# e-sha/dvs_of_training_framework

Hardware: AMD Instinct MI355X
Metric: training samples/sec (256x256x5 event voxels) (higher is better)
Workload: dtype f32; 1 GPU; EV_FlowNet 256x256x5-bin synthetic events, batch 8 per GPU, fp32 (BASELINE.json configs[1]); full step: voxelise + fwd + multi-scale loss + bwd + AdamW-amsgrad; global_batch=8, parallelism=dp1

## Files before the change

dvs_of_training_framework_amd/csrc/fwd_min.hip:

```cpp
#include "conv_common.h"
#include <stdlib.h>

namespace {

constexpr unsigned FM_OOB = 0x80000000u;
constexpr int FM_NT = 512;
constexpr int FM_APA = 5;
constexpr int FM_AP = 8 * FM_APA;
constexpr int FM_AARR = FM_APA * 1024 + 16;

template <int NR>
struct FMGeom {
    static constexpr int PT = NR / 2;
    static constexpr int KS = 8 / PT;
    static constexpr int SLOTS = (NR + 2) * 18;
    static constexpr int BROWS = (SLOTS + 7) / 8;
    static constexpr int BPA = (BROWS + 7) / 8;
    static constexpr int BARR = BPA * 1024 + 16;
    static constexpr int BOFF = 8 * FM_AARR;
    static constexpr int NPIECE = FM_AP + 8 * BPA;
    static constexpr int LPW = NPIECE / 8;
    static constexpr int STAGE = ((8 * FM_AARR + 8 * BARR + 1023) / 1024) * 1024;
    static constexpr int XCH = 8 * 4 * 4096;
    static constexpr int LDS = 2 * STAGE > XCH ? 2 * STAGE : XCH;
};

__global__ __launch_bounds__(256) void min9_fwd_weights_kernel(const float *__restrict__ w, float *__restrict__ wt,
                                                               int Cout, int Ctot)
{
    const size_t i = (size_t)blockIdx.x * 256 + threadIdx.x;
    if (i >= (size_t)Cout * Ctot) return;
    const int ci = (int)(i % Ctot), co = (int)(i / Ctot);
    float k[3][3], r[3][3];
#pragma unroll
    for (int t = 0; t < 9; ++t) k[t / 3][t % 3] = w[((size_t)co * 9 + t) * Ctot + ci];
#pragma unroll
    for (int l = 0; l < 3; ++l) {
        r[0][l] = k[0][l];
        r[1][l] = (k[0][l] + k[1][l]) + k[2][l];
        r[2][l] = k[2][l];
    }
#pragma unroll
    for (int p = 0; p < 3; ++p) {
        const float v[3] = {r[p][0], (r[p][0] + r[p][1]) + r[p][2], r[p][2]};
#pragma unroll
        for (int q = 0; q < 3; ++q) wt[((size_t)(3 * p + q) * Cout + co) * Ctot + ci] = v[q];
    }
}

template <int NR, bool ZOUT>
__global__ __launch_bounds__(FM_NT) void fwd_min_f32_kernel(const GConvParams P)
{
#if defined(__HIP_DEVICE_COMPILE__)
    typedef FMGeom<NR> G;
    typedef float f32x2 __attribute__((ext_vector_type(2)));
    extern __shared__ __attribute__((aligned(1024))) unsigned char smem[];
    const int tid = threadIdx.x, lane = tid & 63;
    const int wave = __builtin_amdgcn_readfirstlane(tid >> 6);
    const int pt = wave % G::PT, ks = wave / G::PT;
    const int lrow = lane & 31, lh = lane >> 5;
    const int H = P.Hv, W = P.Wv;
    const int nbx = W / 16, nby = H / NR;

    unsigned wg = blockIdx.x;
    {
        const unsigned total = gridDim.x, x = wg & 7u, q = total >> 3, r = total & 7u;
        wg = x * q + min(x, r) + (wg >> 3);
    }
    const int nco = P.N / 32;
    const int cot = (int)(wg % (unsigned)nco), blk = (int)(wg / (unsigned)nco);
    const int co0 = 32 * cot;
    const int bx = blk % nbx, by = (blk / nbx) % nby, b = blk / (nbx * nby);
    const int oy = NR * by, ox = 16 * bx;

    const GSrc &S0 = P.src[0], &S1 = P.src[1];
    unsigned off_a[G::LPW], off_b[G::LPW - FM_APA];
#pragma unroll
    for (int i = 0; i < G::LPW; ++i) {
        const int p = wave + 8 * i;
        off_a[i] = FM_OOB;
        if (i >= FM_APA) off_b[i - FM_APA] = FM_OOB;
        if (i < FM_APA) {
            const int m = p / FM_APA, pp = p - FM_APA * m;
            const int j = 8 * pp + (lane >> 3);
            if (j < 36) {
                const int R = 8 * j + m;
                const int c = R >> 5, r = R & 31;
                off_a[i] = (unsigned)((((size_t)c * P.N + co0 + r) * P.Cin_tot + 4 * (lane & 7)) * 4);
            }
        } else {
            const int pb = p - FM_AP;
            const int m = pb / G::BPA, pp = pb - G::BPA * m;
            const int n = 8 * (8 * pp + (lane >> 3)) + m;
            if (n < G::SLOTS) {
                const int r = n / 18, c = n - 18 * r;
                if (((unsigned)(oy + r - 1) < (unsigned)H) & ((unsigned)(ox + c - 1) < (unsigned)W)) {
                    off_a[i] = (unsigned)((r * S0.sy + c * S0.sx + 4 * (lane & 7)) * 4);
                    off_b[i - FM_APA] = (unsigned)((r * S1.sy + c * S1.sx + 4 * (lane & 7)) * 4);
                }
            }
        }
    }
    const __amdgpu_buffer_rsrc_t wres = __builtin_amdgcn_make_buffer_rsrc((void *)P.W, 0, 0x7fffffff, 0x00020000);
    const __amdgpu_buffer_rsrc_t res0 = __builtin_amdgcn_make_buffer_rsrc(
        (void *)(S0.p - ((long long)S0.sy + S0.sx)), 0, 0x7fffffff, 0x00020000);
    const __amdgpu_buffer_rsrc_t res1 = __builtin_amdgcn_make_buffer_rsrc(
        (void *)(S1.p - ((long long)S1.sy + S1.sx)), 0, 0x7fffffff, 0x00020000);
    const int base0 = __builtin_amdgcn_readfirstlane(
        (int)(((long long)b * S0.sb + (long long)oy * S0.sy + (long long)ox * S0.sx) * 4));
    const int base1 = __builtin_amdgcn_readfirstlane(
        (int)(((long long)b * S1.sb + (long long)oy * S1.sy + (long long)ox * S1.sx) * 4));
    const int nch0 = S0.C / 32, nchunks = P.Cin_tot / 32;

    auto issue = [&](int stage_idx, int ch) {
        unsigned char *st = smem + stage_idx * G::STAGE;
        const bool m1 = ch >= nch0;
        const int so_w = ch * 128;
        const int so_x = m1 ? base1 + (ch - nch0) * 128 : base0 + ch * 128;
#pragma unroll
        for (int i = 0; i < G::LPW; ++i) {
            const int p = wave + 8 * i;
            if (i < FM_APA) {
                const int m = p / FM_APA, pp = p - FM_APA * m;
                __attribute__((address_space(3))) void *dst =
                    (__attribute__((address_space(3))) void *)(st + m * FM_AARR + pp * 1024);
                __builtin_amdgcn_raw_ptr_buffer_load_lds(wres, dst, 16, off_a[i], so_w, 0, 0);
            } else {
                const int pb = p - FM_AP;
                const int m = pb / G::BPA, pp = pb - G::BPA * m;
                __attribute__((address_space(3))) void *dst =
                    (__attribute__((address_space(3))) void *)(st + G::BOFF + m * G::BARR + pp * 1024);
                if (m1)
                    __builtin_amdgcn_raw_ptr_buffer_load_lds(res1, dst, 16, off_b[i - FM_APA], so_x, 0, 0);
                else
                    __builtin_amdgcn_raw_ptr_buffer_load_lds(res0, dst, 16, off_a[i], so_x, 0, 0);
            }
        }
    };

#ifndef FM_B64
    constexpr int FRAG = 16;
#else
    constexpr int FRAG = 8;
#endif
    const int abase = (lrow & 7) * FM_AARR + (lrow >> 3) * 128 + FRAG * lh;
    int bbase[9];
#pragma unroll
    for (int r = 0; r < 3; ++r)
#pragma unroll
        for (int c = 0; c < 3; ++c) {
            const int n = (2 * pt + (lrow >> 4) + r) * 18 + (lrow & 15) + c;
            bbase[3 * r + c] = G::BOFF + (n & 7) * G::BARR + (n >> 3) * 128 + FRAG * lh;
        }

    f32x16 acc[9];
#pragma unroll
    for (int c = 0; c < 9; ++c)
#pragma unroll
        for (int r = 0; r < 16; ++r) acc[c][r] = 0.f;

#ifndef FM_PROBE
#define FM_PROBE 0
#endif
    auto compute = [&](int u) {
        const unsigned char *st = smem + u * G::STAGE;
#ifdef FM_STAGGER
        if (wave >= 4) __builtin_amdgcn_s_sleep(FM_STAGGER);
#endif
#ifndef FM_B64
#pragma unroll
        for (int gi = 0; gi < 4 / G::KS; ++gi) {
            const int kg = ks + G::KS * gi;
            f32x4 x[9];
#pragma unroll
            for (int c = 0; c < 9; ++c) x[c] = *(const f32x4 *)(st + bbase[c] + 32 * kg);
            f32x4 an = *(const f32x4 *)(st + abase + 32 * kg);
            f32x4 rw[3][3], xt[9];
#pragma unroll
            for (int c = 0; c < 3; ++c) {
                rw[0][c] = x[c] - x[3 + c];
                rw[1][c] = x[3 + c];
                rw[2][c] = x[6 + c] - x[3 + c];
            }
#pragma unroll
            for (int p = 0; p < 3; ++p) {
                xt[3 * p] = rw[p][0] - rw[p][1];
                xt[3 * p + 1] = rw[p][1];
                xt[3 * p + 2] = rw[p][2] - rw[p][1];
            }
#pragma unroll
            for (int c = 0; c < 9; ++c) {
                const f32x4 ac = an;
                if (c + 1 < 9) an = *(const f32x4 *)(st + abase + (c + 1) * 512 + 32 * kg);
#pragma unroll
                for (int j = 0; j < 4; ++j)
                    acc[c] = __builtin_amdgcn_mfma_f32_32x32x2f32(ac[j], xt[c][j], acc[c], 0, 0, 0);
            }
        }
#else
#pragma unroll
        for (int gi = 0; gi < 8 / G::KS; ++gi) {
            const int kg = ks + G::KS * gi;
            f32x2 a[9], x[9];
#pragma unroll
            for (int c = 0; c < 9; ++c) a[c] = *(const f32x2 *)(st + abase + ((FM_PROBE & 2) ? 0 : c) * 512 + 16 * kg);
#pragma unroll
            for (int c = 0; c < 9; ++c) x[c] = *(const f32x2 *)(st + bbase[(FM_PROBE & 2) ? 0 : c] + 16 * kg);
            f32x2 rw[3][3], xt[9];
#pragma unroll
            for (int c = 0; c < 3; ++c) {
                rw[0][c] = x[c] - x[3 + c];
                rw[1][c] = x[3 + c];
                rw[2][c] = x[6 + c] - x[3 + c];
            }
#pragma unroll
            for (int p = 0; p < 3; ++p) {
                xt[3 * p] = rw[p][0] - rw[p][1];
                xt[3 * p + 1] = rw[p][1];
                xt[3 * p + 2] = rw[p][2] - rw[p][1];
            }
#pragma unroll
            for (int c = 0; c < 9; ++c) {
                acc[c] = __builtin_amdgcn_mfma_f32_32x32x2f32(a[c][0], xt[c][0], acc[c], 0, 0, 0);
                acc[c] = __builtin_amdgcn_mfma_f32_32x32x2f32(a[c][1], xt[c][1], acc[c], 0, 0, 0);
            }
        }
#endif
    };

    issue(0, 0);
    for (int ch = 0; ch < nchunks; ++ch) {
        asm volatile("s_waitcnt vmcnt(0)" ::: "memory");
        if (!(FM_PROBE & 4) || ch == 0) __builtin_amdgcn_s_barrier();
        if (ch + 1 < nchunks && (!(FM_PROBE & 1) || ch == 0)) issue((ch + 1) & 1, ch + 1);
        compute(ch & 1);
    }

    const int ecq = lane & 7;
    f32x4 bias4 = {0.f, 0.f, 0.f, 0.f};
    if (P.bias) bias4 = *(const f32x4 *)(P.bias + co0 + 4 * ecq);
    __builtin_amdgcn_s_barrier();
#pragma unroll
    for (int f = 0; f < 4; ++f) {
        const int fa = f >> 1, fb = f & 1;
        const f32x16 t = (acc[3 * fa + fb] + acc[3 * fa + fb + 1]) + (acc[3 * fa + 3 + fb] + acc[3 * fa + 4 + fb]);
        unsigned char *xt_ = smem + (wave * 4 + f) * 4096;
#pragma unroll
        for (int g = 0; g < 4; ++g) {
            const f32x4 v = {t[4 * g], t[4 * g + 1], t[4 * g + 2], t[4 * g + 3]};
            *(f32x4 *)(xt_ + lrow * 128 + (((2 * g + lh) ^ (lrow & 7)) << 4)) = v;
        }
    }
    __builtin_amdgcn_s_barrier();
    const GDst &D = P.dst[0];
#pragma unroll
    for (int fi = 0; fi < 4 / G::KS; ++fi) {
        const int f = ks + G::KS * fi;
        const int fa = f >> 1, fb = f & 1;
#pragma unroll
        for (int it = 0; it < 4; ++it) {
            const int px = 8 * it + (lane >> 3);
            const int xo = px * 128 + ((ecq ^ (px & 7)) << 4);
            f32x4 v = *(const f32x4 *)(smem + (pt * 4 + f) * 4096 + xo);
#pragma unroll
            for (int k = 1; k < G::KS; ++k) v += *(const f32x4 *)(smem + ((pt + G::PT * k) * 4 + f) * 4096 + xo);
            const int yy = oy + 2 * pt + (px >> 4), xx = ox + (px & 15);
            const long long o = (long long)b * D.sb + (long long)yy * D.sy + (long long)xx * D.sx +
                                (long long)fa * D.ph_y + (long long)fb * D.ph_x + co0 + 4 * ecq;
            v += bias4;
            if (P.bias_cls) {
                const int Y = 2 * yy + fa, X = 2 * xx + fb;
                const int cls = 3 * (Y == 0 ? 1 : Y == P.out_H - 1 ? 2 : 0) + (X == 0 ? 1 : X == P.out_W - 1 ? 2 : 0);
                if (cls) v += *(const f32x4 *)(P.bias_cls + cls * P.N + co0 + 4 * ecq);
            }
            if (ZOUT) *(f32x4 *)(P.zout + o) = v;
#pragma unroll
            for (int e = 0; e < 4; ++e) v[e] = act_fwd(v[e], P.act);
            *(f32x4 *)(D.p + o) = v;
        }
    }
#endif
}

}

bool min9_shape_ok(int mfma, int nsrc, const int *C, const int *nhwc, int Cout, int H, int W)
{
    static const bool off = getenv("DVSOF_NO_FWD_MIN") != nullptr;
    if (off || mfma != 0 || nsrc != 2) return false;
    for (int s = 0; s < 2; ++s)
        if (!nhwc[s] || (C[s] & 31)) return false;
    return (Cout & 31) == 0 && (W % 16) == 0 && (H % 4) == 0 && H >= 4;
}

int min9_prepare_fwd(const float *w, float *wt, int Cout, int Ctot, hipStream_t st)
{
    const size_t n = (size_t)Cout * Ctot;
    hipLaunchKernelGGL(min9_fwd_weights_kernel, dim3((unsigned)((n + 255) / 256)), dim3(256), 0, st, w, wt, Cout, Ctot);
    DVSOF_LAUNCH_CHECK();
    return DVSOF_OK;
}

template <int NR, bool ZOUT>
static int fm_launch(const GConvParams &P, int grid, hipStream_t st)
{
    typedef FMGeom<NR> G;
    static bool attr_set = false;
    if (!attr_set) {
        DVSOF_HIP_TRY(hipFuncSetAttribute((const void *)fwd_min_f32_kernel<NR, ZOUT>,
                                          hipFuncAttributeMaxDynamicSharedMemorySize, G::LDS));
        attr_set = true;
    }
    hipLaunchKernelGGL((fwd_min_f32_kernel<NR, ZOUT>), dim3(grid), dim3(FM_NT), G::LDS, st, P);
    DVSOF_LAUNCH_CHECK();
    conv_note_kernel(NR == 8 ? DVSOF_KERNEL_FWD_MIN8 : DVSOF_KERNEL_FWD_MIN4, 0);
    return DVSOF_OK;
}

int fwd_min_launch(const GConvParams &P, hipStream_t st)
{
    for (int s = 0; s < 2; ++s) {
        const GSrc &S = P.src[s];
        if (!S.p || (reinterpret_cast<uintptr_t>(S.p) & 15) || ((S.sb | S.sy | S.sx) & 3) || S.sc != 1) return DVSOF_EINVAL;
    }
    const GDst &D = P.dst[0];
    if (D.addend || D.addend2 || D.actsrc || D.sc != 1 || ((D.sb | D.sy | D.sx | D.ph_y | D.ph_x) & 3)) return DVSOF_EINVAL;
    if ((reinterpret_cast<uintptr_t>(D.p) & 15) || (reinterpret_cast<uintptr_t>(P.zout) & 15) ||
        (reinterpret_cast<uintptr_t>(P.W) & 15) || (reinterpret_cast<uintptr_t>(P.bias) & 15) ||
        (reinterpret_cast<uintptr_t>(P.bias_cls) & 15))
        return DVSOF_EINVAL;
    static const int force = getenv("DVSOF_FWD_MIN_NR") ? atoi(getenv("DVSOF_FWD_MIN_NR")) : 0;
    const long long per_row = (long long)P.B * (P.Wv / 16) * (P.N / 32);
    int nr = 4;
    if (P.Hv % 8 == 0 && per_row * (P.Hv / 8) >= 256) nr = 8;
    if ((force == 4 || force == 8) && P.Hv % force == 0) nr = force;
    const int grid = (int)(per_row * (P.Hv / nr));
    const bool z = P.zout != nullptr;
    if (nr == 8) return z ? fm_launch<8, true>(P, grid, st) : fm_launch<8, false>(P, grid, st);
    return z ? fm_launch<4, true>(P, grid, st) : fm_launch<4, false>(P, grid, st);
}
```

Baseline: 3263 samples/s.

## Stage 16-channel chunks through a four-deep LDS ring with software-pipelined MFMA

Shrinks each staged channel chunk from 32 to 16 channels and replaces the two-stage double buffer with a four-slot LDS ring, issuing loads two chunks ahead and waiting with a counted vmcnt instead of draining all loads. The compute is split into a load/Winograd-transform step and an MFMA step, and some waves lag the MFMA by one chunk so transforms and matrix work from different chunks interleave across waves. The weight and patch layouts in LDS are rebuilt for 4-row interleaving. This aims to hide global-to-LDS latency and barrier stalls, at the cost of more iterations, more barriers per channel, and more complex indexing that could introduce layout or bank-conflict issues.

```diff
diff --git a/dvs_of_training_framework_amd/csrc/fwd_min.hip b/dvs_of_training_framework_amd/csrc/fwd_min.hip
--- a/dvs_of_training_framework_amd/csrc/fwd_min.hip
+++ b/dvs_of_training_framework_amd/csrc/fwd_min.hip
@@ -5,24 +5,24 @@
 
 constexpr unsigned FM_OOB = 0x80000000u;
 constexpr int FM_NT = 512;
-constexpr int FM_APA = 5;
-constexpr int FM_AP = 8 * FM_APA;
-constexpr int FM_AARR = FM_APA * 1024 + 16;
+constexpr int FM_RING = 4;
+constexpr int FM_LPW = 4;
+constexpr int FM_STAGE = 8 * FM_LPW * 1024;
+constexpr int FM_AROWS = 72;
+constexpr int FM_AARR = FM_AROWS * 64 + 16;
+constexpr int FM_BOFF = ((4 * FM_AARR + 1023) / 1024) * 1024;
+constexpr int FM_WP = FM_BOFF / 1024;
 
 template <int NR>
 struct FMGeom {
     static constexpr int PT = NR / 2;
     static constexpr int KS = 8 / PT;
     static constexpr int SLOTS = (NR + 2) * 18;
-    static constexpr int BROWS = (SLOTS + 7) / 8;
-    static constexpr int BPA = (BROWS + 7) / 8;
-    static constexpr int BARR = BPA * 1024 + 16;
-    static constexpr int BOFF = 8 * FM_AARR;
-    static constexpr int NPIECE = FM_AP + 8 * BPA;
-    static constexpr int LPW = NPIECE / 8;
-    static constexpr int STAGE = ((8 * FM_AARR + 8 * BARR + 1023) / 1024) * 1024;
+    static constexpr int BROWS = ((SLOTS + 3) / 4 + 3) / 4 * 4;
+    static constexpr int BARR = BROWS * 64 + 16;
+    static_assert(FM_BOFF + 4 * BARR <= FM_STAGE, "the patch image overflows the stage");
     static constexpr int XCH = 8 * 4 * 4096;
-    static constexpr int LDS = 2 * STAGE > XCH ? 2 * STAGE : XCH;
+    static constexpr int LDS = FM_RING * FM_STAGE > XCH ? FM_RING * FM_STAGE : XCH;
 };
 
 __global__ __launch_bounds__(256) void min9_fwd_weights_kernel(const float *__restrict__ w, float *__restrict__ wt,
@@ -53,7 +53,6 @@
 {
 #if defined(__HIP_DEVICE_COMPILE__)
     typedef FMGeom<NR> G;
-    typedef float f32x2 __attribute__((ext_vector_type(2)));
     extern __shared__ __attribute__((aligned(1024))) unsigned char smem[];
     const int tid = threadIdx.x, lane = tid & 63;
     const int wave = __builtin_amdgcn_readfirstlane(tid >> 6);
@@ -74,29 +73,29 @@
     const int oy = NR * by, ox = 16 * bx;
 
     const GSrc &S0 = P.src[0], &S1 = P.src[1];
-    unsigned off_a[G::LPW], off_b[G::LPW - FM_APA];
-#pragma unroll
-    for (int i = 0; i < G::LPW; ++i) {
+    unsigned off_a[FM_LPW], off_b[FM_LPW];
+#pragma unroll
+    for (int i = 0; i < FM_LPW; ++i) {
         const int p = wave + 8 * i;
+        const int a = 1024 * p + 16 * lane;
         off_a[i] = FM_OOB;
-        if (i >= FM_APA) off_b[i - FM_APA] = FM_OOB;
-        if (i < FM_APA) {
-            const int m = p / FM_APA, pp = p - FM_APA * m;
-            const int j = 8 * pp + (lane >> 3);
-            if (j < 36) {
-                const int R = 8 * j + m;
+        off_b[i] = FM_OOB;
+        if (p < FM_WP) {
+            const int m = a / FM_AARR, o = a - FM_AARR * m;
+            if (m < 4 && o < FM_AROWS * 64) {
+                const int R = 4 * (o >> 6) + m;
                 const int c = R >> 5, r = R & 31;
-                off_a[i] = (unsigned)((((size_t)c * P.N + co0 + r) * P.Cin_tot + 4 * (lane & 7)) * 4);
+                off_a[i] = (unsigned)((((size_t)c * P.N + co0 + r) * P.Cin_tot + 4 * ((o >> 4) & 3)) * 4);
             }
         } else {
-            const int pb = p - FM_AP;
-            const int m = pb / G::BPA, pp = pb - G::BPA * m;
-            const int n = 8 * (8 * pp + (lane >> 3)) + m;
-            if (n < G::SLOTS) {
-                const int r = n / 18, c = n - 18 * r;
+            const int ab = a - FM_BOFF;
+            const int m = ab / G::BARR, o = ab - G::BARR * m;
+            const int n = 4 * (o >> 6) + m;
+            if (m < 4 && o < G::BROWS * 64 && n < G::SLOTS) {
+                const int r = n / 18, c = n - 18 * r, qq = (o >> 4) & 3;
                 if (((unsigned)(oy + r - 1) < (unsigned)H) & ((unsigned)(ox + c - 1) < (unsigned)W)) {
-                    off_a[i] = (unsigned)((r * S0.sy + c * S0.sx + 4 * (lane & 7)) * 4);
-                    off_b[i - FM_APA] = (unsigned)((r * S1.sy + c * S1.sx + 4 * (lane & 7)) * 4);
+                    off_a[i] = (unsigned)((r * S0.sy + c * S0.sx + 4 * qq) * 4);
+                    off_b[i] = (unsigned)((r * S1.sy + c * S1.sx + 4 * qq) * 4);
                 }
             }
         }
@@ -110,47 +109,35 @@
         (int)(((long long)b * S0.sb + (long long)oy * S0.sy + (long long)ox * S0.sx) * 4));
     const int base1 = __builtin_amdgcn_readfirstlane(
         (int)(((long long)b * S1.sb + (long long)oy * S1.sy + (long long)ox * S1.sx) * 4));
-    const int nch0 = S0.C / 32, nchunks = P.Cin_tot / 32;
-
-    auto issue = [&](int stage_idx, int ch) {
-        unsigned char *st = smem + stage_idx * G::STAGE;
+    const int nch0 = S0.C / 16, nchunks = P.Cin_tot / 16;
+
+    auto issue = [&](int u, int ch) {
+        unsigned char *st = smem + u * FM_STAGE;
         const bool m1 = ch >= nch0;
-        const int so_w = ch * 128;
-        const int so_x = m1 ? base1 + (ch - nch0) * 128 : base0 + ch * 128;
-#pragma unroll
-        for (int i = 0; i < G::LPW; ++i) {
+        const int so_w = __builtin_amdgcn_readfirstlane(ch * 64);
+        const int so_x = __builtin_amdgcn_readfirstlane(m1 ? base1 + (ch - nch0) * 64 : base0 + ch * 64);
+#pragma unroll
+        for (int i = 0; i < FM_LPW; ++i) {
             const int p = wave + 8 * i;
-            if (i < FM_APA) {
-                const int m = p / FM_APA, pp = p - FM_APA * m;
-                __attribute__((address_space(3))) void *dst =
-                    (__attribute__((address_space(3))) void *)(st + m * FM_AARR + pp * 1024);
+            __attribute__((address_space(3))) void *dst = (__attribute__((address_space(3))) void *)(st + 1024 * p);
+            if (p < FM_WP)
                 __builtin_amdgcn_raw_ptr_buffer_load_lds(wres, dst, 16, off_a[i], so_w, 0, 0);
-            } else {
-                const int pb = p - FM_AP;
-                const int m = pb / G::BPA, pp = pb - G::BPA * m;
-                __attribute__((address_space(3))) void *dst =
-                    (__attribute__((address_space(3))) void *)(st + G::BOFF + m * G::BARR + pp * 1024);
-                if (m1)
-                    __builtin_amdgcn_raw_ptr_buffer_load_lds(res1, dst, 16, off_b[i - FM_APA], so_x, 0, 0);
-                else
-                    __builtin_amdgcn_raw_ptr_buffer_load_lds(res0, dst, 16, off_a[i], so_x, 0, 0);
-            }
+            else if (m1)
+                __builtin_amdgcn_raw_ptr_buffer_load_lds(res1, dst, 16, off_b[i], so_x, 0, 0);
+            else
+                __builtin_amdgcn_raw_ptr_buffer_load_lds(res0, dst, 16, off_a[i], so_x, 0, 0);
         }
     };
 
-#ifndef FM_B64
-    constexpr int FRAG = 16;
-#else
-    constexpr int FRAG = 8;
-#endif
-    const int abase = (lrow & 7) * FM_AARR + (lrow >> 3) * 128 + FRAG * lh;
+    const int kl = ks & 1;
+    const int abase = (lrow & 3) * FM_AARR + (lrow >> 2) * 64 + 16 * lh + 32 * kl;
     int bbase[9];
 #pragma unroll
     for (int r = 0; r < 3; ++r)
 #pragma unroll
         for (int c = 0; c < 3; ++c) {
             const int n = (2 * pt + (lrow >> 4) + r) * 18 + (lrow & 15) + c;
-            bbase[3 * r + c] = G::BOFF + (n & 7) * G::BARR + (n >> 3) * 128 + FRAG * lh;
+            bbase[3 * r + c] = FM_BOFF + (n & 3) * G::BARR + (n >> 2) * 64 + 16 * lh + 32 * kl;
         }
 
     f32x16 acc[9];
@@ -162,79 +149,59 @@
 #ifndef FM_PROBE
 #define FM_PROBE 0
 #endif
-    auto compute = [&](int u) {
-        const unsigned char *st = smem + u * G::STAGE;
-#ifdef FM_STAGGER
-        if (wave >= 4) __builtin_amdgcn_s_sleep(FM_STAGGER);
-#endif
-#ifndef FM_B64
-#pragma unroll
-        for (int gi = 0; gi < 4 / G::KS; ++gi) {
-            const int kg = ks + G::KS * gi;
-            f32x4 x[9];
-#pragma unroll
-            for (int c = 0; c < 9; ++c) x[c] = *(const f32x4 *)(st + bbase[c] + 32 * kg);
-            f32x4 an = *(const f32x4 *)(st + abase + 32 * kg);
-            f32x4 rw[3][3], xt[9];
-#pragma unroll
-            for (int c = 0; c < 3; ++c) {
-                rw[0][c] = x[c] - x[3 + c];
-                rw[1][c] = x[3 + c];
-                rw[2][c] = x[6 + c] - x[3 + c];
-            }
-#pragma unroll
-            for (int p = 0; p < 3; ++p) {
-                xt[3 * p] = rw[p][0] - rw[p][1];
-                xt[3 * p + 1] = rw[p][1];
-                xt[3 * p + 2] = rw[p][2] - rw[p][1];
-            }
-#pragma unroll
-            for (int c = 0; c < 9; ++c) {
-                const f32x4 ac = an;
-                if (c + 1 < 9) an = *(const f32x4 *)(st + abase + (c + 1) * 512 + 32 * kg);
-#pragma unroll
-                for (int j = 0; j < 4; ++j)
-                    acc[c] = __builtin_amdgcn_mfma_f32_32x32x2f32(ac[j], xt[c][j], acc[c], 0, 0, 0);
-            }
-        }
-#else
-#pragma unroll
-        for (int gi = 0; gi < 8 / G::KS; ++gi) {
-            const int kg = ks + G::KS * gi;
-            f32x2 a[9], x[9];
-#pragma unroll
-            for (int c = 0; c < 9; ++c) a[c] = *(const f32x2 *)(st + abase + ((FM_PROBE & 2) ? 0 : c) * 512 + 16 * kg);
-#pragma unroll
-            for (int c = 0; c < 9; ++c) x[c] = *(const f32x2 *)(st + bbase[(FM_PROBE & 2) ? 0 : c] + 16 * kg);
-            f32x2 rw[3][3], xt[9];
-#pragma unroll
-            for (int c = 0; c < 3; ++c) {
-                rw[0][c] = x[c] - x[3 + c];
-                rw[1][c] = x[3 + c];
-                rw[2][c] = x[6 + c] - x[3 + c];
-            }
-#pragma unroll
-            for (int p = 0; p < 3; ++p) {
-                xt[3 * p] = rw[p][0] - rw[p][1];
-                xt[3 * p + 1] = rw[p][1];
-                xt[3 * p + 2] = rw[p][2] - rw[p][1];
-            }
-#pragma unroll
-            for (int c = 0; c < 9; ++c) {
-                acc[c] = __builtin_amdgcn_mfma_f32_32x32x2f32(a[c][0], xt[c][0], acc[c], 0, 0, 0);
-                acc[c] = __builtin_amdgcn_mfma_f32_32x32x2f32(a[c][1], xt[c][1], acc[c], 0, 0, 0);
-            }
-        }
-#endif
+
+    auto load = [&](int u, f32x4 (&xt)[9]) {
+        const unsigned char *st = smem + u * FM_STAGE;
+        f32x4 x[9];
+#pragma unroll
+        for (int c = 0; c < 9; ++c) x[c] = *(const f32x4 *)(st + bbase[(FM_PROBE & 2) ? 0 : c]);
+        f32x4 rw[3][3];
+#pragma unroll
+        for (int c = 0; c < 3; ++c) {
+            rw[0][c] = x[c] - x[3 + c];
+            rw[1][c] = x[3 + c];
+            rw[2][c] = x[6 + c] - x[3 + c];
+        }
+#pragma unroll
+        for (int p = 0; p < 3; ++p) {
+            xt[3 * p] = rw[p][0] - rw[p][1];
+            xt[3 * p + 1] = rw[p][1];
+            xt[3 * p + 2] = rw[p][2] - rw[p][1];
+        }
     };
-
+    auto mma = [&](int u, const f32x4 (&xt)[9]) {
+        const unsigned char *st = smem + u * FM_STAGE;
+        f32x4 an = *(const f32x4 *)(st + abase);
+#pragma unroll
+        for (int c = 0; c < 9; ++c) {
+            const f32x4 ac = an;
+            if (c + 1 < 9) an = *(const f32x4 *)(st + abase + ((FM_PROBE & 2) ? 0 : (c + 1) * 512));
+#pragma unroll
+            for (int j = 0; j < 4; ++j)
+                acc[c] = __builtin_amdgcn_mfma_f32_32x32x2f32(ac[j], xt[c][j], acc[c], 0, 0, 0);
+        }
+    };
+
+    const bool lag = !(FM_PROBE & 8) && (G::KS == 4 || wave >= 4);
+    const int par = ks >> 1;
+    f32x4 xt[9];
     issue(0, 0);
-    for (int ch = 0; ch < nchunks; ++ch) {
-        asm volatile("s_waitcnt vmcnt(0)" ::: "memory");
-        if (!(FM_PROBE & 4) || ch == 0) __builtin_amdgcn_s_barrier();
-        if (ch + 1 < nchunks && (!(FM_PROBE & 1) || ch == 0)) issue((ch + 1) & 1, ch + 1);
-        compute(ch & 1);
-    }
+    if (nchunks > 1) issue(1, 1);
+    static_assert(FM_LPW == 4, "the counted wait below");
+    for (int t = 0; t < nchunks; ++t) {
+        if (t + 1 < nchunks) asm volatile("s_waitcnt vmcnt(4)" ::: "memory");
+        else asm volatile("s_waitcnt vmcnt(0)" ::: "memory");
+        if (!(FM_PROBE & 4) || t == 0) __builtin_amdgcn_s_barrier();
+        asm volatile("" ::: "memory");
+        if (t + 2 < nchunks && !(FM_PROBE & 1)) issue((t + 2) & 3, t + 2);
+        const bool mine = G::KS == 2 || (t & 1) == par;
+        if (lag && t > 0 && (G::KS == 2 || !mine)) mma((t - 1) & 3, xt);
+        if (mine) {
+            load(t & 3, xt);
+            if (!lag) mma(t & 3, xt);
+        }
+    }
+    if (lag && (G::KS == 2 || ((nchunks - 1) & 1) == par)) mma((nchunks - 1) & 3, xt);
 
     const int ecq = lane & 7;
     f32x4 bias4 = {0.f, 0.f, 0.f, 0.f};
```

Measured after the change: 3210 samples/s, median of 2. 0.984x the previous value.
